# TzuYaoHuang/WaterLily.jl

Measured on AMD Instinct MI355X. Metric: cells*steps/sec (3D TGV) ; smoother HBM GB/s vs peak, higher is better.
Workload: dtype f32; 1 GPU; 3D Taylor-Green vortex 512^3 Float32, wall-bounded, Re=1600, NoBody, remeasure=false (BASELINE configs[4] domain on 1 GPU); size=512, resjac=630, resjac_redo=0

## Files before the change

waterlily.jl_amd/csrc/wl_common.hpp:

```cpp
#pragma once
#include <functional>
#include <cstdlib>
#include <hip/hip_runtime.h>
#include <stdint.h>

#include <mutex>
#include <string>
#include <vector>

#include "../../include/wlhip.h"
#include "../../include/wlhip_bench.h"

#define WL_WAVE 64
#define WL_BLOCK 256

void wl_set_error(const std::string& s);
#define WL_HIP(call)                                                                      \
  do {                                                                                    \
    hipError_t e__ = (call);                                                              \
    if (e__ != hipSuccess) {                                                              \
      wl_set_error(std::string(#call) + ": " + hipGetErrorString(e__));                   \
      return (int)e__;                                                                    \
    }                                                                                     \
  } while (0)
// ... 121 lines not shown
  RedWs w; char* b = (char*)base;
  w.pa = (double*)b; w.pb = (double*)(b + (size_t)WL_MAXPART * 8); w.pm = (float*)(b + (size_t)WL_MAXPART * 16);
  w.res_d = (double*)(b + (size_t)WL_MAXPART * 20); w.res_f = (float*)(b + (size_t)WL_MAXPART * 20 + 64);
  return w;
}

struct WlCtx {
  bool inited = false;
  int device = 0;
  void* red = nullptr;
  double* h_d = nullptr;
  float* h_f = nullptr;
};
WlCtx& wl_ctx();
int wl_ctx_ensure();

struct WlProf {
  bool on = false;
  bool only_roofline = false;
  struct Slot { std::vector<hipEvent_t> a, b; size_t used = 0; };
  Slot slot[WL_PROF_NSLOTS];
};
WlProf& wl_prof();
struct ProfScope {
  int id; hipStream_t s; bool active; size_t idx;
  ProfScope(int id_, hipStream_t s_);
  ~ProfScope();
};

struct BcFold { int on; float U[3];
                const float* proj_x = nullptr; int proj_done = 0;
                int usub = 0;
                const float* go = nullptr;
                const float* dt_dev = nullptr; };

namespace wl {
struct ConstL { int on; float c[3]; float Dt[27]; float iDt[27]; };
#ifdef __HIPCC__
__device__ __forceinline__ float wl_cl_coef(int Ia, int Na, float c) { return (Ia <= 2 || Ia >= Na) ? 0.f : c; }
__device__ __forceinline__ int wl_cl_cnt(int Ia, int Na) { return ((Ia <= 2 || Ia >= Na) ? 0 : 1) + ((Ia + 1 <= 2 || Ia + 1 >= Na) ? 0 : 1); }
#endif
int check_const_L(const float* L, const GridX& g, ConstL* out, int* dev_flag, hipStream_t s);
int const_plane_range(const float* L, const GridX& g, const float* c, int* za, int* zb, hipStream_t s);
int fill(float* a, float v, size_t n, hipStream_t s);
int scale(float* a, float s_, size_t n, hipStream_t s);
int div_scalar(float* a, float s_, size_t n, hipStream_t s);
int div_scalar_to(float* out, const float* in, float s_, size_t n, hipStream_t s);
int sum_dev(const float* a, size_t n, const RedWs& ws, int slot, hipStream_t s);
int l1_linf_dev(const float* a, size_t n, const RedWs& ws, int slot_d, int slot_f, hipStream_t s);
int max_dev(const float* a, size_t n, const RedWs& ws, int slot_f, hipStream_t s);
int dot_dev(const float* a, const float* b, size_t n, const RedWs& ws, int slot, hipStream_t s);
int read_results(const RedWs& ws, double* hd, int nd, float* hf, int nf, hipStream_t s);
int read_results_overlapped(const RedWs& ws, double* hd, int nd, float* hf, int nf, hipStream_t s, hipEvent_t copied, const std::function<int()>& queue_behind);
std::mutex& wl_read_mutex();

int bc_vec(float* a, const GridX& g, const float* U, int saveexit, unsigned per, hipStream_t s);
int bc_per_scalar(float* a, const GridX& g, unsigned per, hipStream_t s);
int conv_diff(float* r, const float* u, float* Phi, const GridX& g, float nu, unsigned per, int scheme, hipStream_t s);
int conv_diff_bdim(float* f, const float* u_adv, float* Phi, const float* u0, const float* mu0, float* u_out, const GridX& g, float nu, unsigned per, int scheme,
                   float dt, float pre, float post, const ConstL& cl, hipStream_t s, int ka = -(1 << 30), int kb = 1 << 30, bool q1 = true, BcFold* fold = nullptr);
int conv_q1(float* Phi, const float* u, const GridX& g, float nu, unsigned per, int scheme, hipStream_t s);
bool conv_z_ok(const GridX& g, unsigned per);
int conv_diff_z(float* f, const float* u_adv, const float* u0, const float* mu0, float* u_out, const GridX& g, float nu, int scheme, float dt, float pre, float post, hipStream_t s);
int bdim(float* u, const float* u0, float* f, const float* V, const float* mu0, const float* mu1, const GridX& g, float dt, float pre, float post, hipStream_t s);
int accelerate(float* r, const GridX& g, const float* a, hipStream_t s);
int sgs(float* f, float* sigma, const float* u, const GridX& g, float Cs, float Delta, hipStream_t s);
int bc_vec_fn(float* a, const float* Ub, const GridX& g, int saveexit, unsigned per, hipStream_t s);
// ... 97 lines not shown
```

waterlily.jl_amd/csrc/wl_poisson.hip:

```cpp
#include <vector>

#include "wl_common.hpp"
#include "wl_bcfold.hpp"
#include "wl_pdefer.hpp"

namespace {

__device__ __forceinline__ bool cell_ij(const GridX& g, long m, int& i, int& j) {
  if (m >= g.sz) return false;
  j = (int)(m / g.nx);
  i = (int)(m - (long)j * g.nx);
  return true;
}
__device__ __forceinline__ bool interior_ij(const GridX& g, int i, int j) { return i >= 1 && i <= g.nx - 2 && j >= 1 && j <= g.ny - 2; }

template <int D>
__device__ __forceinline__ float Ax(const GridX& g, long o, const float* __restrict__ L, const float* __restrict__ Dg, const float* __restrict__ x) {
  float s = x[o] * Dg[o];
  s += (x[o - 1] * L[o] + x[o + 1] * L[o + 1]);
  s += (x[o - g.sy] * L[g.cs + o] + x[o + g.sy] * L[g.cs + o + g.sy]);
  if (D == 3) s += (x[o - g.sz] * L[2 * g.cs + o] + x[o + g.sz] * L[2 * g.cs + o + g.sz]);
  return s;
}

// ... 255 lines not shown
      if (bc.usub) {
        if (i0 == 0 || i0 == g.nx - 2) a0.y = bc.U[0];
        if (j == 1) a1 = make_float2(bc.U[1], bc.U[1]);
        if (j + 1 == g.ny - 1) a1p = make_float2(bc.U[1], bc.U[1]);
        if (g.gk + k == 1) a2 = make_float2(bc.U[2], bc.U[2]);
        if (g.gk + k + 1 == g.gnz - 1) a2p = make_float2(bc.U[2], bc.U[2]);
      }
      const float uxn0 = a0.x - lx0 * (xc.x - xl), uxp0 = a0.y - lx1 * (xc.y - xc.x);
      const float uyn0 = a1.x - ly * (xc.x - xym.x), uyp0 = a1p.x - lyp * (xyp.x - xc.x);
      const float uzn0 = a2.x - lz * (xc.x - xzm.x), uzp0 = a2p.x - lzp * (xzp.x - xc.x);
      const float uxn1 = a0.y - lx1 * (xc.y - xc.x), uxp1 = axr - lx2 * (xr - xc.y);
      const float uyn1 = a1.y - ly * (xc.y - xym.y), uyp1 = a1p.y - lyp * (xyp.y - xc.y);
      const float uzn1 = a2.y - lz * (xc.y - xzm.y), uzp1 = a2p.y - lzp * (xzp.y - xc.y);
      if (in0) { sg0 = 0.f; sg0 += (fmaxf(0.f, uxp0) + fmaxf(0.f, -uxn0)); sg0 += (fmaxf(0.f, uyp0) + fmaxf(0.f, -uyn0)); sg0 += (fmaxf(0.f, uzp0) + fmaxf(0.f, -uzn0)); }
      if (in1) { sg1 = 0.f; sg1 += (fmaxf(0.f, uxp1) + fmaxf(0.f, -uxn1)); sg1 += (fmaxf(0.f, uyp1) + fmaxf(0.f, -uyn1)); sg1 += (fmaxf(0.f, uzp1) + fmaxf(0.f, -uzn1)); }
      const float va[3] = {uxn0, uyn0, uzn0}, vb[3] = {uxn1, uyn1, uzn1};
      const bool plain0 = !bc.on || wl_bc_fold_plain(g, i0, j, k), plain1 = !bc.on || wl_bc_fold_plain(g, i0 + 1, j, k);
      if (in0 && in1 && plain0 && plain1) { pl_st2(uout, o, make_float2(va[0], vb[0])); pl_st2(uout, g.cs + o, make_float2(va[1], vb[1])); pl_st2(uout, 2 * g.cs + o, make_float2(va[2], vb[2])); }
      else {
        if (in0) { if (plain0) { uout[o] = va[0]; uout[g.cs + o] = va[1]; uout[2 * g.cs + o] = va[2]; } else wl_bc_fold_store(uout, g, i0, j, k, va, bc.U); }
        if (in1) { if (plain1) { uout[o + 1] = vb[0]; uout[g.cs + o + 1] = vb[1]; uout[2 * g.cs + o + 1] = vb[2]; } else wl_bc_fold_store(uout, g, i0 + 1, j, k, vb, bc.U); }
      }
      if (store_sigma) { if (in0) sigma[o] = sg0; if (in1) sigma[o + 1] = sg1; }
    }
    if (want) {
      if (!in0) sg0 = sigma[o];
      if (!in1) sg1 = sigma[o + 1];
      mx = fmaxf(sg0, sg1);
    }
  }
  mx = block_max(mx);
  if (threadIdx.x == 0) atomicMax(reinterpret_cast<int*>(pmax) + (blockIdx.x & (WL_ENC_SLOTS - 1)), wl_enc_f(mx));
}

__global__ void k_fin_max_enc(const int* __restrict__ p, float* __restrict__ om) {
  float mx = -INFINITY;
  for (int q = threadIdx.x; q < WL_ENC_SLOTS; q += WL_BLOCK) { const int k = p[q]; if (k != (int)0x80000000) mx = fmaxf(mx, wl_dec_f(k)); }
  mx = block_max(mx); if (threadIdx.x == 0) *om = mx;
}
__global__ void k_fin_max2(const float* __restrict__ pmax, int n, float* __restrict__ om) {
  float mx = -INFINITY, m1 = -INFINITY, m2 = -INFINITY, m3 = -INFINITY;
  int q = threadIdx.x;
  for (; q + 3 * WL_BLOCK < n; q += 4 * WL_BLOCK) { mx = fmaxf(mx, pmax[q]); m1 = fmaxf(m1, pmax[q + WL_BLOCK]); m2 = fmaxf(m2, pmax[q + 2 * WL_BLOCK]); m3 = fmaxf(m3, pmax[q + 3 * WL_BLOCK]); }
  for (; q < n; q += WL_BLOCK) mx = fmaxf(mx, pmax[q]);
  mx = fmaxf(fmaxf(mx, m1), fmaxf(m2, m3));
  mx = block_max(mx); if (threadIdx.x == 0) *om = mx;
}
template <int D>
__global__ void k_check_const_L(GridX g, const float* __restrict__ L, float c0, float c1, float c2, int* __restrict__ flag) {
  int i, j; long m; int pz;
  wl_tile(g, m, pz);
  if (!cell_ij(g, m, i, j)) return;
  const int k = pz;
  const int Kj = (D == 3) ? g.gk + k + 1 : 1;
  if (D == 3 && (Kj < 1 || Kj > g.gnz)) return;
  if (D == 3 && g.nz != g.gnz && (k < g.k0 - 1 || k > g.k1)) return;
  const long o = m + (long)k * g.sz;
  const float c[3] = {c0, c1, c2};
  const int I[3] = {i + 1, j + 1, Kj};
  const int N[3] = {g.nx, g.ny, (D == 3) ? g.gnz : 1};
  bool bad = false;
  for (int a = 0; a < D; a++) {
    const float want = (I[a] <= 2 || I[a] >= N[a]) ? 0.f : c[a];
    bad = bad || (L[(long)a * g.cs + o] != want);
  }
  if (bad) atomicOr(flag, 1);
// ... 648 lines not shown
  hipLaunchKernelGGL(k_final_sum, dim3(1), dim3(WL_BLOCK), 0, s, ws.pa, (int)grid.x, ws.res_d + 0);
  WL_LAUNCH_CHECK(); return 0;
}
#define DSEL2(D, CLF, KERN, ...)                                                                                     \
  do { if ((D) == 3) { if (CLF) hipLaunchKernelGGL((KERN<3, 1>), __VA_ARGS__); else hipLaunchKernelGGL((KERN<3, 0>), __VA_ARGS__); } \
       else { if (CLF) hipLaunchKernelGGL((KERN<2, 1>), __VA_ARGS__); else hipLaunchKernelGGL((KERN<2, 0>), __VA_ARGS__); } } while (0)
int div_residual(float* z, float* xout, float* r, const float* x, const float* u, const float* L, const float* Dg, const float* iD, const GridX& g, float dt, const RedWs& ws, const ConstL& cl, hipStream_t s) {
  const int zc = wl_march_chunk(g, g.nz);
  dim3 grid = wl_plane_grid(g, wl_march_slots(g.nz, zc));
  DSEL2(g.D, cl.on, k_div_residual, grid, dim3(WL_BLOCK), 0, s, g, z, xout, r, x, u, L, Dg, iD, dt, ws.pa, cl, zc, 0, g.nz);
  hipLaunchKernelGGL(k_final_sum, dim3(1), dim3(WL_BLOCK), 0, s, ws.pa, (int)grid.x, ws.res_d + 0);
  WL_LAUNCH_CHECK(); return 0;
}
int div_residual_split(float* z, float* xout, float* r, const float* x, const float* u, const float* L, const float* Dg, const float* iD, const GridX& g, float dt, const RedWs& ws,
                       const ConstL& near, const ConstL& far, int na, int nb, hipStream_t s) {
  const int lo[3] = {0, na, nb}, hi[3] = {na, nb, g.nz};
  int off = 0;
  for (int q = 0; q < 3; q++) {
    const int np = hi[q] - lo[q];
    if (np <= 0) continue;
    const ConstL& cl = q == 1 ? near : far;
    const int zc = wl_march_chunk(g, np);
    dim3 grid = wl_plane_grid(g, wl_march_slots(np, zc));
    if (off + (int)grid.x > WL_MAXPART) { wl_set_error("div_residual_split: too many partial sums"); return WL_EINVAL; }
    DSEL2(g.D, cl.on, k_div_residual, grid, dim3(WL_BLOCK), 0, s, g, z, xout, r, x, u, L, Dg, iD, dt, ws.pa + off, cl, zc, lo[q], hi[q]);
    off += (int)grid.x;
  }
  hipLaunchKernelGGL(k_final_sum, dim3(1), dim3(WL_BLOCK), 0, s, ws.pa, off, ws.res_d + 0);
  WL_LAUNCH_CHECK(); return 0;
}
static int tail_pair_bits() { static const int v = wl_exp_int("WL_TAIL_PAIR", 2); return v; }
static int tail_pair() { return tail_pair_bits() & 1; }
static int tail_lin(int bit) { static const int v = wl_exp_int("WL_TAIL_LIN", 1); return (v >> bit) & 1; }
int project_unscale(float* u, const float* L, const float* x, float* pout, const GridX& g, float dt, const ConstL& cl, hipStream_t s, const BcFold* fold) {
  return project_unscale(u, L, x, pout, g, dt, cl, s, fold, false);
}
int project_unscale(float* u, const float* L, const float* x, float* pout, const GridX& g, float dt, const ConstL& cl, hipStream_t s, const BcFold* fold, bool skip_p) {
  const int lin = tail_lin(0) && g.D == 3;
  const int zc = lin ? 1 : wl_march_chunk(g, g.nz);
  BcFold bc{0, {0.f, 0.f, 0.f}};
  if (fold && fold->on && g.D == 3 && g.nz == g.gnz && g.nx >= 6 && g.ny >= 6 && g.nz >= 6) bc = *fold;
  bc.go = fold ? fold->go : nullptr;
  if (tail_pair() && lin && cl.on && (g.nx & 1) == 0 && g.k0 >= 1) {
    if (skip_p) hipLaunchKernelGGL(k_project_unscale2<0>, dim3(pl_grid(g, g.nz)), dim3(WL_BLOCK), 0, s, g, u, x, pout, dt, cl, 0, g.nz, bc);
    else hipLaunchKernelGGL(k_project_unscale2<1>, dim3(pl_grid(g, g.nz)), dim3(WL_BLOCK), 0, s, g, u, x, pout, dt, cl, 0, g.nz, bc);
    WL_LAUNCH_CHECK(); return 0;
  }
  if (skip_p) {
    if (!(g.D == 3 && cl.on)) { wl_set_error("project_unscale: the tail without the p store needs a 3-D constant-coefficient level"); return WL_EINVAL; }
    hipLaunchKernelGGL((k_project_unscale<3, 1, 0>), wl_plane_grid(g, wl_march_slots(g.nz, zc)), dim3(WL_BLOCK), 0, s, g, u, L, x, pout, dt, cl, zc, 0, g.nz, bc, lin);
    WL_LAUNCH_CHECK(); return 0;
  }
  DSEL2(g.D, cl.on, k_project_unscale, wl_plane_grid(g, wl_march_slots(g.nz, zc)), dim3(WL_BLOCK), 0, s, g, u, L, x, pout, dt, cl, zc, 0, g.nz, bc, lin);
  WL_LAUNCH_CHECK(); return 0;
}
int project_unscale_split(float* u, const float* L, const float* x, float* pout, const GridX& g, float dt, const ConstL& near, const ConstL& far, int na, int nb, hipStream_t s) {
  const int lo[3] = {0, na, nb}, hi[3] = {na, nb, g.nz};
  for (int q = 0; q < 3; q++) {
    const int np = hi[q] - lo[q];
    if (np <= 0) continue;
    const ConstL& cl = q == 1 ? near : far;
    const int zc = wl_march_chunk(g, np);
    DSEL2(g.D, cl.on, k_project_unscale, wl_plane_grid(g, wl_march_slots(np, zc)), dim3(WL_BLOCK), 0, s, g, u, L, x, pout, dt, cl, zc, lo[q], hi[q], BcFold{0, {0.f, 0.f, 0.f}}, 0);
  }
  WL_LAUNCH_CHECK(); return 0;
}
__global__ void k_decide(const double* __restrict__ res_d, float* __restrict__ res_f, double r1tol, double rinftol, double ninside, int check_head, int slot_d, int slot_f, int out_slot) {
  const float rnew = (float)res_d[slot_d], rinf = res_f[slot_f];
  const bool ok = (double)rnew < r1tol && (double)rinf < rinftol;
  const bool head_due = check_head == 2 || (check_head == 1 && wl_shift_due(res_d[0], ninside));
  res_f[out_slot] = head_due ? -1.f : (ok ? 1.f : 0.f);
}
int decide_converged(const RedWs& ws, double r1tol, double rinftol, double ninside, int check_head, int slot_d, int slot_f, int out_slot, hipStream_t s) {
  hipLaunchKernelGGL(k_decide, dim3(1), dim3(1), 0, s, (const double*)ws.res_d, ws.res_f, r1tol, rinftol, ninside, check_head, slot_d, slot_f, out_slot);
  WL_LAUNCH_CHECK(); return 0;
}
bool project_cfl_pair_path(const GridX& g, const ConstL& cl) { return (tail_pair_bits() & 2) && g.D == 3 && cl.on && (g.nx & 1) == 0 && g.k0 >= 1 && g.k1 <= g.nz - 1; }
int project_cfl(float* uout, const float* uin, const float* L, const float* x, float* pout, float* sigma, const GridX& g, float dt, const ConstL& cl, const RedWs& ws, int slot_f, hipStream_t s, int store_sigma, const BcFold* fold) {
  return project_cfl(uout, uin, L, x, pout, sigma, g, dt, cl, ws, slot_f, s, store_sigma, fold, false);
}
int project_cfl(float* uout, const float* uin, const float* L, const float* x, float* pout, float* sigma, const GridX& g, float dt, const ConstL& cl, const RedWs& ws, int slot_f, hipStream_t s, int store_sigma, const BcFold* fold,
                bool skip_p) {
  if (uout == uin) { wl_set_error("project_cfl: output aliases input"); return WL_EINVAL; }
  int kfirst = 0, klast = 1;
  if (g.D == 3) { kfirst = (g.gk + g.k0 == 1) ? g.k0 - 1 : g.k0; klast = (g.gk + g.k1 == g.gnz - 1) ? g.k1 + 1 : g.k1; }
  BcFold bc{0, {0.f, 0.f, 0.f}};
  if (fold && fold->on && g.D == 3 && g.nz == g.gnz && g.nx >= 6 && g.ny >= 6 && g.nz >= 6) bc = *fold;
  bc.go = fold ? fold->go : nullptr;
  if (bc.go && !project_cfl_pair_path(g, cl)) { wl_set_error("project_cfl: a tail queued ahead of the convergence read needs the two-cells-per-thread form"); return WL_EINVAL; }
  if (fold && fold->usub && !(bc.on && project_cfl_pair_path(g, cl))) { wl_set_error("project_cfl: deferred BC! needs the folded two-cells-per-thread tail"); return WL_EINVAL; }
  if (skip_p && !project_cfl_pair_path(g, cl)) { wl_set_error("project_cfl: the tail without the p store needs the two-cells-per-thread form"); return WL_EINVAL; }
  if (project_cfl_pair_path(g, cl)) {
    hipLaunchKernelGGL(k_enc_init, dim3(1), dim3(WL_ENC_SLOTS), 0, s, reinterpret_cast<int*>(ws.pm));
    if (skip_p) hipLaunchKernelGGL(k_project_cfl2<0>, dim3(pl_grid(g, g.nz)), dim3(WL_BLOCK), 0, s, g, uout, uin, x, pout, sigma, dt, cl, kfirst, klast, ws.pm, 0, g.nz, store_sigma, bc);
    else hipLaunchKernelGGL(k_project_cfl2<1>, dim3(pl_grid(g, g.nz)), dim3(WL_BLOCK), 0, s, g, uout, uin, x, pout, sigma, dt, cl, kfirst, klast, ws.pm, 0, g.nz, store_sigma, bc);
    hipLaunchKernelGGL(k_fin_max_enc, dim3(1), dim3(WL_BLOCK), 0, s, reinterpret_cast<const int*>(ws.pm), ws.res_f + slot_f);
    WL_LAUNCH_CHECK(); return 0;
  }
  const int lin = tail_lin(1) && g.D == 3;
  const int zc = lin ? 1 : wl_march_chunk(g, g.nz);
  const dim3 grid = wl_plane_grid(g, wl_march_slots(g.nz, zc));
  if (lin) hipLaunchKernelGGL(k_enc_init, dim3(1), dim3(WL_ENC_SLOTS), 0, s, reinterpret_cast<int*>(ws.pm));
  DSEL2(g.D, cl.on, k_project_cfl, grid, dim3(WL_BLOCK), 0, s, g, uout, uin, L, x, pout, sigma, dt, cl, zc, kfirst, klast, ws.pm, 0, g.nz, store_sigma, bc, lin);
  if (lin) hipLaunchKernelGGL(k_fin_max_enc, dim3(1), dim3(WL_BLOCK), 0, s, reinterpret_cast<const int*>(ws.pm), ws.res_f + slot_f);
  else hipLaunchKernelGGL(k_fin_max2, dim3(1), dim3(WL_BLOCK), 0, s, ws.pm, (int)grid.x, ws.res_f + slot_f);
  WL_LAUNCH_CHECK(); return 0;
}
int project_cfl_split(float* uout, const float* uin, const float* L, const float* x, float* pout, float* sigma, const GridX& g, float dt, const ConstL& near, const ConstL& far,
                      int na, int nb, const RedWs& ws, int slot_f, hipStream_t s, int store_sigma) {
  if (uout == uin) { wl_set_error("project_cfl: output aliases input"); return WL_EINVAL; }
  int kfirst = 0, klast = 1;
  if (g.D == 3) { kfirst = (g.gk + g.k0 == 1) ? g.k0 - 1 : g.k0; klast = (g.gk + g.k1 == g.gnz - 1) ? g.k1 + 1 : g.k1; }
  const int lo[3] = {0, na, nb}, hi[3] = {na, nb, g.nz};
  int off = 0;
  for (int q = 0; q < 3; q++) {
    const int np = hi[q] - lo[q];
    if (np <= 0) continue;
    const ConstL& cl = q == 1 ? near : far;
    const int zc = wl_march_chunk(g, np);
    const dim3 grid = wl_plane_grid(g, wl_march_slots(np, zc));
    if (off + (int)grid.x > WL_MAXPART) { wl_set_error("project_cfl_split: too many partial maxima"); return WL_EINVAL; }
    DSEL2(g.D, cl.on, k_project_cfl, grid, dim3(WL_BLOCK), 0, s, g, uout, uin, L, x, pout, sigma, dt, cl, zc, kfirst, klast, ws.pm + off, lo[q], hi[q], store_sigma, BcFold{0, {0.f, 0.f, 0.f}}, 0);
    off += (int)grid.x;
  }
  hipLaunchKernelGGL(k_fin_max2, dim3(1), dim3(WL_BLOCK), 0, s, ws.pm, off, ws.res_f + slot_f);
  WL_LAUNCH_CHECK(); return 0;
}
// ... 172 lines not shown
```

waterlily.jl_amd/csrc/wl_sim.hip:

```cpp
#include <cmath>
#include <cstring>
#include <utility>
#include <vector>

#include "wl_common.hpp"
#include <algorithm>
#include "wl_mg.hpp"
#include "wl_body.hpp"
#include "wl_pdefer.hpp"

namespace {
__device__ __forceinline__ bool cell_ij(const GridX& g, long m, int& i, int& j) {
  if (m >= g.sz) return false;
  j = (int)(m / g.nx);
  i = (int)(m - (long)j * g.nx);
  return true;
}
__device__ __forceinline__ bool interior_ij(const GridX& g, int i, int j) { return i >= 1 && i <= g.nx - 2 && j >= 1 && j <= g.ny - 2; }

template <int D>
__global__ void k_apply_tgv(GridX g, float* __restrict__ u, float kx, float ky, float kz) {
  int i, j; long m; int pz;
  wl_tile(g, m, pz);
  if (!cell_ij(g, m, i, j)) return;
// ... 370 lines not shown
          WL_TRY(sync_u(s));
          WL_TRY(wl::conv_diff_z(store_f ? f : nullptr, u, u0, mu0, us, G, d.nu, d.scheme, dt.back(), 1.f, 0.5f, s));
          WL_TRY(wl::conv_q1(sigma, u, G, d.nu, d.perdir_mask, d.scheme, s));
        } else { WL_TRY(conv_fused(u, us, 1.f, 0.5f, s)); fused_conv = true; } }
      std::swap(u, us);
      if (d.exitBC) WL_TRY(copy_exit_face(u, us, s));
      return fused_conv ? bc_u_or_defer(true, s) : bc_u(s);
    }
    { ProfScope pc(WL_PROF_CONVDIFF, s); WL_TRY(conv_only(u, s)); }
    WL_TRY(sgs_udf(u, s));
    if (forcing) WL_TRY(wl::accelerate(f, G, acc1, s));
    WL_TRY(bdim_step(1.f, 0.5f, s));
    return bc_u(s);
  }
  int itmx = 32;
  bool use_resjac = true;
  bool use_headspec = true;
  bool resjac_force_redo = false;
  bool redo_unannounced = false;
  long n_tailfuse = 0;
  long n_resjac = 0, n_resjac_redo = 0;
  int resjac_redo_run = 0;
  bool resjac_backoff = false;
  int p_shell = -1;
  bool use_fuse_cfl = true;
  bool cfl_done = false;
  static constexpr int CFL_SLOT = 5;
  bool use_tailspec = true;
  long n_tailspec = 0, n_tailspec_armed = 0;
  bool use_pdefer = true;
  float p_scale_pending = 0.f;
  long n_pdefer = 0;
  float* p_home = nullptr;
  bool pdefer_ok() const { return use_pdefer && in_step && !sgs_model && !forcing && !d.has_body && head_fused_ok(); }
  int materialise_p(hipStream_t s) {
    if (p_scale_pending == 0.f) return 0;
    const float dp = p_scale_pending; p_scale_pending = 0.f;
    WL_TRY(wl::div_scalar_to(ps, p, dp, (size_t)G.cs, s));
    std::swap(p, ps); mg->lv[0].x = p;
    return 0;
  }
  int project(float w, hipStream_t s, bool with_cfl = false, bool defer_tail = false, bool more_follow = false) {
    const float dtl = w * dt.back();
    cfl_done = false;
    if (p_scale_pending != 0.f && !head_fused_ok()) WL_TRY(materialise_p(s));
    WL_TRY(sync_u(s));
    if (bc_deferred && !head_fused_ok()) WL_TRY(flush_bc(s));
    if (ps && use_fuse_p && !(comm && d.perdir_mask)) {
      WL_TRY(wl::bc_per_scalar(p, G, d.perdir_mask, s));
      wl_mg::Level& l0 = mg->lv[0];
      bool head_done = false;
      double pre_r1 = 0.0; float pre_rinf = 0.f;
      bool solved = false;
      const bool split = l0.part && mg->use_zsplit && !comm;
      const int zm = 4, zna = split ? std::max(l0.g.k0, l0.za - zm) : 0, znb = split ? std::min(l0.g.k1, l0.zb + zm + 1) : 0;
      int tail_kind = 0;
      bool tail_stood = false;
      bool tail_skips_p = false;
      auto skip_p_now = [&]() -> bool {
        if (!pdefer_ok()) return false;
        if (with_cfl) return more_follow;
        if (!defer_tail) return false;
        return !p_home || more_follow || p == p_home;
      };
      auto launch_tail = [&](const float* go) -> int {
        tail_skips_p = false;
        if (with_cfl && use_fuse_cfl && us && !d.exitBC && !d.perdir_mask) {
          tail_kind = 1;
          if (split) { WL_TRY(flush_bc(s)); WL_TRY(wl::project_cfl_split(us, u, mu0, p, ps, sigma, G, dtl, l0.cl, l0.clp, zna, znb, mg->ws, CFL_SLOT, s, store_f ? 1 : 0)); }
          else {
            BcFold fr = fold_req(1);
            if (bc_deferred && !(fr.on && wl::project_cfl_pair_path(G, l0.cl))) WL_TRY(flush_bc(s));
            fr.usub = bc_deferred ? 1 : 0;
            fr.go = go;
            tail_skips_p = wl::project_cfl_pair_path(G, l0.cl) && skip_p_now();
            WL_TRY(wl::project_cfl(us, u, mu0, p, ps, sigma, G, dtl, l0.cl, mg->ws, CFL_SLOT, s, store_f ? 1 : 0, &fr, tail_skips_p)); bc_folded = fr.on != 0;
          }
        } else if (split) { tail_kind = 2; WL_TRY(wl::project_unscale_split(u, mu0, p, ps, G, dtl, l0.cl, l0.clp, zna, znb, s)); }
        else if (defer_tail && tailfuse_ok()) {
          tail_kind = 3;
          tail_skips_p = skip_p_now();
          if (!tail_skips_p) WL_TRY(wl::div_scalar_to(ps, p, dtl, (size_t)G.cs, s));
        }
        else { tail_kind = 2; BcFold fr = fold_req(1); fr.go = go; tail_skips_p = skip_p_now(); WL_TRY(wl::project_unscale(u, mu0, p, ps, G, dtl, l0.cl, s, &fr, tail_skips_p)); bc_folded = fr.on != 0; }
        return 0;
      };
      const bool tail_gateable = !split && !(defer_tail && tailfuse_ok()) &&
                                 (!(with_cfl && use_fuse_cfl && us && !d.exitBC && !d.perdir_mask) || (wl::project_cfl_pair_path(G, l0.cl) && (!bc_deferred || fold_req(1).on)));
      if (use_resjac && !resjac_backoff && !d.exitBC && !store_f && !d.perdir_mask && !l0.part && mg->defer_shift && mg->lv.size() > 1 && wl::resjac_ok(G, l0.cl) &&
          (!comm || (l0.dist && mg->x_halo_depth >= 2))) {
        { ProfScope pr(WL_PROF_RESIDUAL, s);
          if (comm) p_shell = 1;
          if (p_shell < 0) p_shell = (wl::shell_nonzero(p, G, (int*)(mg->ws.res_f + 7), s) || wl::shell_nonzero(ps, G, (int*)(mg->ws.res_f + 7), s)) ? 1 : 0;
          WL_TRY(wl::resjac(ps, l0.eps, p, u, G, dtl, 1.f, l0.cl, mg->ws, 1, 0, s, p_shell != 0, bc_deferred ? d.uBC : nullptr, p_scale_pending)); }
        if (use_headspec && !comm && itmx >= 1) {
          std::swap(p, ps); l0.x = p;
          std::swap(l0.r, l0.eps);
          mg->jacobi0_done = true;
          struct SpecClear { wl_mg* m; ~SpecClear() { m->spec_tail = nullptr; m->spec_check_head = 0; } } spec_clear{mg};
          if (use_tailspec && tail_gateable) { mg->spec_tail = launch_tail; mg->spec_check_head = resjac_force_redo ? 2 : 1; n_tailspec_armed++; }
          WL_TRY(mg->solve(2e-3, itmx, nullptr, nullptr, nullptr, s, true, nullptr, nullptr));
          tail_stood = mg->tail_stood; if (tail_stood) n_tailspec++;
          const bool due = mg->head_decided ? mg->head_due : (resjac_force_redo || wl_shift_due(mg->first_hd0, (double)wl_ninside_global(mg->lv[0].g)));
          if (!due) { head_done = true; solved = true; n_resjac++; resjac_redo_run = 0; }
          else {
            std::swap(l0.r, l0.eps); std::swap(p, ps); l0.x = p;
            mg->n.pop_back(); mg->jacobi0_done = false;
            n_resjac_redo++;
            if (!resjac_force_redo && ++resjac_redo_run >= 3) resjac_backoff = true;
          }
        } else {
        WL_TRY(wl::combine_results(comm, mg->ws, s));
        double hd2[2]; WL_TRY(wl::read_results(mg->ws, hd2, 2, &pre_rinf, 1, s));
        const double sr = hd2[0]; pre_r1 = hd2[1];
        if (!wl_shift_due(sr, (double)wl_ninside_global(mg->lv[0].g)) && !resjac_force_redo) {
          std::swap(p, ps); l0.x = p;
          std::swap(l0.r, l0.eps);
          mg->jacobi0_done = true; head_done = true; n_resjac++; resjac_redo_run = 0;
        } else {
          n_resjac_redo++;
          if (!resjac_force_redo && ++resjac_redo_run >= 3) resjac_backoff = true;
        }
        }
      }
      if (head_done) p_scale_pending = 0.f;
      if (!head_done) {
        WL_TRY(materialise_p(s));
        WL_TRY(flush_bc(s));
        ProfScope pr(WL_PROF_RESIDUAL, s);
        if (l0.part && mg->use_zsplit && !comm) {
          const int m = 4, na = std::max(l0.g.k0, l0.za - m), nb = std::min(l0.g.k1, l0.zb + m + 1);
          WL_TRY(wl::div_residual_split(store_f ? sigma : nullptr, ps, l0.r, p, u, mu0, l0.D, l0.iD, G, dtl, mg->ws, l0.cl, l0.clp, na, nb, s));
        } else WL_TRY(wl::div_residual(store_f ? sigma : nullptr, ps, l0.r, p, u, mu0, l0.D, l0.iD, G, dtl, mg->ws, l0.cl, s));
      }
      if (!head_done) { std::swap(p, ps); l0.x = p; }
      if (!solved) WL_TRY(mg->solve(2e-3, itmx, nullptr, nullptr, nullptr, s, true, head_done ? &pre_r1 : nullptr, head_done ? &pre_rinf : nullptr));
      if (!tail_stood) WL_TRY(launch_tail(nullptr));
      if (tail_kind == 3) {
        bc_deferred = false;
        proj_pending = p;
        if (tail_skips_p) { p_scale_pending = dtl; n_pdefer++; }
        else { std::swap(p, ps); l0.x = p; }
        n_tailfuse++;
        return 0;
      }
      if (tail_kind == 1) {
        bc_deferred = false;
        WL_TRY(wl::combine_results(comm, mg->ws, s));
        std::swap(u, us); cfl_done = true;
      }
      if (tail_skips_p) { p_scale_pending = dtl; n_pdefer++; }
      else { std::swap(p, ps); l0.x = p; }
      bc_deferred = false;
      return bc_u(s);
    }
    WL_TRY(materialise_p(s));
    WL_TRY(flush_bc(s));
    WL_TRY(wl::div_scale(sigma, p, u, G, dtl, s));
    WL_TRY(mg->solve(2e-3, itmx, nullptr, nullptr, nullptr, s));
    WL_TRY(wl::project(u, mu0, p, G, s));
    WL_TRY(wl::div_scalar(p, dtl, (size_t)G.cs, s));
    return bc_u(s);
  }
  bool use_lazydt = true, dt_pending = false;
  hipEvent_t ev_dt = nullptr;
  bool lazydt_ok() const {
    return use_lazydt && in_step && !comm && us && !d.has_body && !forcing && !sgs_model && !use_convz && !d.exitBC && !d.perdir_mask && !store_f && wl::conv_flux_on() &&
           wl::conv_tile_ok(G, d.perdir_mask, G.k1 - G.k0) && mg->lv[0].cl.on;
  }
  int cfl(hipStream_t s, bool more_follow = false) {
    if (!cfl_done) { WL_TRY(sync_u(s)); WL_TRY(wl::cfl_dev(u, sigma, G, mg->ws, CFL_SLOT, s)); WL_TRY(wl::combine_results(comm, mg->ws, s)); }
    cfl_done = false;
    if (more_follow && lazydt_ok()) {
      hipLaunchKernelGGL(k_dt_from_cfl, dim3(1), dim3(1), 0, s, mg->ws.res_f, CFL_SLOT, CFL_SLOT + 1, d.nu);
      dt_pending = true;
      return 0;
    }
    float hf6[CFL_SLOT + 1]; WL_TRY(wl::read_results(mg->ws, nullptr, 0, hf6, CFL_SLOT + 1, s)); const float mx = hf6[CFL_SLOT];
    dt.push_back(std::fmin(10.f, 1.0f / (mx + 5 * d.nu)));
    return 0;
  }
  int mom_step(hipStream_t s, bool more_follow = false) {
    const int rc = mom_step_body(s, more_follow);
// ... 220 lines not shown
  const std::string n(name);
  if (n == "convz") { s->use_convz = value != 0; return 0; }
  if (n == "fused_smoother") { s->mg->use_fused = value != 0; return 0; }
  if (n == "store_eps") { s->mg->store_eps = value != 0; return 0; }
  if (n == "constl") { s->mg->use_constl = value != 0; return s->mg->update(0); }
  if (n == "tail") { s->mg->use_tail = value != 0; return 0; }
  if (n == "tail_lds") { wl::tail_lds_enable(value); return 0; }
  if (n == "xdefer") { s->mg->use_xdefer = value != 0; return 0; }
  if (n == "overlap_smooth") { s->mg->overlap_smooth = value != 0; return 0; }
  if (n == "body_tile") { wl::conv_body_tile_enable(value); return 0; }
  if (n == "skip_fill") { s->mg->skip_fill = value != 0; return 0; }
  if (n == "defer_shift") { s->mg->defer_shift = value != 0; return 0; }
  if (n == "zsplit") {
    s->mg->use_zsplit = value != 0; s->mg->zsplit_min = value == 2 ? 0 : (value >= 4 ? (long)value << 20 : 16L << 20); return 0;
  }
  if (n == "hybrid") { s->use_hybrid = value != 0; return 0; }
  if (n == "farmask") { s->use_farmask = value != 0; return 0; }
  if (n == "store_f") { s->store_f = value != 0; return 0; }
  if (n == "overlap") { WL_TRY(s->sync_u(0)); s->use_overlap = value != 0; return 0; }
  if (n == "fuse_cfl") { s->use_fuse_cfl = value != 0; return 0; }
  if (n == "jacobi_march") { wl::jacobi_march_enable(value); return 0; }
  if (n == "convm") { wl::conv_march_enable(value); return 0; }
  if (n == "deep_halo") { s->mg->deep_halo = value != 0; return 0; }
  if (n == "x_halo") { if (value < 1 || value > s->G.k0) { wl_set_error("x_halo: 1 .. ghost depth of the slab"); return WL_EINVAL; } s->mg->x_halo_depth = value; return 0; }
  if (n == "bcfold") { s->use_bcfold = value; return 0; }
  if (n == "resjac") { s->use_resjac = value != 0; s->resjac_force_redo = value == 2 || value == 3; s->redo_unannounced = value == 3; return 0; }
  if (n == "resjac_min") { wl::resjac_enable(1, value); return 0; }
  if (n == "convt_min") { wl::conv_tile_min(value); return 0; }
  if (n == "lazydt") { s->use_lazydt = value != 0; return 0; }
  if (n == "tailspec") { s->use_tailspec = value != 0; return 0; }
  if (n == "headspec") { s->use_headspec = value != 0; return 0; }
  if (n == "bcdefer") { s->use_bcdefer = value != 0; return 0; }
  if (n == "pdefer") { s->use_pdefer = value != 0; return 0; }
  if (n == "tailfuse") { s->use_tailfuse = value != 0; return 0; }
  if (n == "convf") { wl::conv_flux_enable(value != 0); return 0; }
  if (n == "convt") { wl::conv_tile_enable(value != 0, value > 1 ? value : 0); return 0; }
  if (n == "pair") { wl::gsrb_pair_enable(value); return 0; }
  if (n == "fuse_p") { s->use_fuse_p = value != 0; return 0; }
  if (n == "zsplit_par") { s->mg->par_ranges = value != 0; return 0; }
  if (n == "itmx") { if (value < 1) { wl_set_error("itmx must be >= 1"); return WL_EINVAL; } s->itmx = value; return 0; }
  wl_set_error("unknown option " + n); return WL_EINVAL;
}
int wl_sim_update(wl_sim* s, void* st) { s->resjac_backoff = false; s->resjac_redo_run = 0; WL_TRY(s->refresh_body_mask(wl_stream(st))); return s->mg->update(wl_stream(st)); }

long wl_launch_count(void) { return g_wl_launches; }
int wl_reset_process_options(void) {
  wl::resjac_enable(1, 6L << 20); wl::conv_tile_min(2048); wl::conv_tile_enable(1, 0); wl::conv_flux_enable(1); wl::tail_lds_enable(1); wl::conv_body_tile_enable(1);
  wl::gsrb_pair_enable(1); wl::jacobi_march_enable(1); wl::conv_march_enable(0);
  return 0;
}
int wl_sim_counter(wl_sim* s, const char* name, long* out) {
  WL_CHECK(s && name && out, "bad argument");
  const std::string n(name);
  if (n == "resjac") { *out = s->n_resjac; return 0; }
  if (n == "resjac_redo") { *out = s->n_resjac_redo; return 0; }
  if (n == "resjac_backoff") { *out = s->resjac_backoff ? 1 : 0; return 0; }
  if (n == "tailfuse") { *out = s->n_tailfuse; return 0; }
  if (n == "bcdefer") { *out = s->n_bcdefer; return 0; }
  if (n == "pdefer") { *out = s->n_pdefer; return 0; }
  if (n == "tailspec") { *out = s->n_tailspec; return 0; }
  if (n == "tailspec_armed") { *out = s->n_tailspec_armed; return 0; }
  if (n == "xdefer") { *out = s->mg->last_xdefer; return 0; }
  wl_set_error("unknown counter " + n); return WL_EINVAL;
}
int wl_sim_set_forcing(wl_sim* s, const float* U1, const float* a0, const float* a1) {
  const int D = s->d.D;
  if (U1) for (int c = 0; c < D; c++) s->d.uBC[c] = U1[c];
  s->forcing = a0 != nullptr || a1 != nullptr;
  for (int c = 0; c < 3; c++) { s->acc0[c] = (a0 && c < D) ? a0[c] : 0.f; s->acc1[c] = (a1 && c < D) ? a1[c] : 0.f; }
  return 0;
}
int wl_sim_set_sgs(wl_sim* s, int model, float Cs, float Delta) {
  WL_CHECK(s, "null wl_sim"); WL_CHECK(model == 0 || model == 1, "wl_sim_set_sgs: model must be 0 (off) or 1 (Smagorinsky-Lilly)");
  if (model) {
    if (s->d.D != 3) { wl_set_error("wl_sim_set_sgs: the Smagorinsky model is built for 3-D flows only"); return WL_EINVAL; }
    if (s->comm) { wl_set_error("wl_sim_set_sgs: z-slab handles are not supported (single domain only)"); return WL_EINVAL; }
  }
  s->sgs_model = model; s->sgs_Cs = Cs; s->sgs_Delta = Delta;
  return 0;
}
int wl_accelerate(float* r, const wl_grid* g, const float* a, void* st) {
  WL_CHECK(wl_grid_ok(g) && a, "bad argument"); WL_TRY(wl_ctx_ensure());
  return wl::accelerate(r, gx(*g), a, wl_stream(st));
}
int wl_sim_mom_step(wl_sim* s, void* st) { return s->mom_step(wl_stream(st)); }
int wl_sim_mom_steps(wl_sim* s, int n, void* st) {
  WL_CHECK(s && n >= 0, "bad argument");
  for (int k = 0; k < n; k++) WL_TRY(s->mom_step(wl_stream(st), k + 1 < n));
  return 0;
}
int wl_sim_dt(const wl_sim* s, float* out, int cap) { const int n = (int)s->dt.size(); for (int k = 0; k < n && k < cap; k++) out[k] = s->dt[(size_t)k]; return n; }
float wl_sim_dt_last(const wl_sim* s) { return s->dt.back(); }
// ... 157 lines not shown
```

Before: 14.51 billion cells*steps/s.

## Add four-cells-per-thread projection tail kernel with LDS-staged pressure plane

Adds a new projection/CFL tail kernel in which each thread handles four consecutive cells using float4 loads and stores. The pressure chunk plus its y-halo is staged in shared memory so the x and y neighbours are read from LDS instead of global memory. It is enabled by default through a new tailwide option and is guarded by alignment and shape checks. The aim is fewer memory transactions and better bandwidth use in the once-per-step tail. In exchange it uses LDS and more registers, has more complex boundary handling, and can fall back to the older paired kernel.

```diff
diff --git a/waterlily.jl_amd/csrc/wl_common.hpp b/waterlily.jl_amd/csrc/wl_common.hpp
--- a/waterlily.jl_amd/csrc/wl_common.hpp
+++ b/waterlily.jl_amd/csrc/wl_common.hpp
@@ -177,7 +177,8 @@
                 const float* proj_x = nullptr; int proj_done = 0;
                 int usub = 0;
                 const float* go = nullptr;
-                const float* dt_dev = nullptr; };
+                const float* dt_dev = nullptr;
+                int wide = 0; int* wide_ran = nullptr; };
 
 namespace wl {
 struct ConstL { int on; float c[3]; float Dt[27]; float iDt[27]; };
diff --git a/waterlily.jl_amd/csrc/wl_poisson.hip b/waterlily.jl_amd/csrc/wl_poisson.hip
--- a/waterlily.jl_amd/csrc/wl_poisson.hip
+++ b/waterlily.jl_amd/csrc/wl_poisson.hip
@@ -311,6 +311,130 @@
   mx = block_max(mx);
   if (threadIdx.x == 0) atomicMax(reinterpret_cast<int*>(pmax) + (blockIdx.x & (WL_ENC_SLOTS - 1)), wl_enc_f(mx));
 }
+#define WL_TW_CHUNK (4 * WL_BLOCK)
+__device__ __forceinline__ float4 tw_ld4(const float* __restrict__ p, long o) { return *reinterpret_cast<const float4*>(p + o); }
+__device__ __forceinline__ void tw_st4(float* __restrict__ p, long o, float4 v) { *reinterpret_cast<float4*>(p + o) = v; }
+static inline unsigned tw_nb8(const GridX& g) { const long nb = (g.sz + WL_TW_CHUNK - 1) / WL_TW_CHUNK; return (unsigned)(((nb + 7) >> 3) << 3); }
+static inline unsigned tw_grid(const GridX& g, int nplanes) { return tw_nb8(g) * (unsigned)nplanes; }
+static inline size_t tw_lds_bytes(const GridX& g) { return (size_t)(WL_TW_CHUNK + 2 * g.sy + 8) * sizeof(float); }
+template <int CFL, int SP>
+__global__ void __launch_bounds__(WL_BLOCK) k_project_wide(GridX g, float* __restrict__ uout, const float* __restrict__ uin, const float* __restrict__ x, float* __restrict__ pout,
+                                                              float* __restrict__ sigma, float dt, wl::ConstL cl, int kfirst, int klast, float* __restrict__ pmax, int p0, int p1,
+                                                              int store_sigma, BcFold bc, unsigned nb8) {
+  if (bc.go && !(*bc.go > 0.f)) return;
+  extern __shared__ float4 tw_sh[];
+  float* __restrict__ xs = reinterpret_cast<float*>(tw_sh);
+  const float* __restrict__ ui = CFL ? uin : uout;
+  const unsigned h = blockIdx.x, p = h / nb8;
+  const int k = p0 + (int)p;
+  const long m0 = (long)(h - p * nb8) * WL_TW_CHUNK;
+  float mx = -INFINITY;
+  if (m0 < g.sz && k < p1) {
+    const long ko = (long)k * g.sz;
+    const int sy = (int)g.sy;
+    const long base = (m0 - sy) & ~3L;
+    const bool zin = k >= g.k0 && k < g.k1;
+    if (zin) {
+      const long whi = (m0 + WL_TW_CHUNK + (CFL ? sy : 0) + 3) & ~3L;
+      for (long q = base + 4 * (long)threadIdx.x; q < whi; q += 4 * WL_BLOCK)
+        *reinterpret_cast<float4*>(xs + (q - base)) = (q >= 0 && q < g.sz) ? tw_ld4(x, ko + q) : make_float4(0.f, 0.f, 0.f, 0.f);
+      __syncthreads();
+    }
+    const float lz = wl::wl_cl_coef(g.gk + k + 1, g.gnz, cl.c[2]), lzp = wl::wl_cl_coef(g.gk + k + 2, g.gnz, cl.c[2]);
+    const bool want = CFL && k >= kfirst && k < klast;
+    const long m = m0 + 4 * (long)threadIdx.x;
+    if (m < g.sz) {
+      const long o = ko + m;
+      const int r = (int)(m - base);
+      const float4 xq = zin ? *reinterpret_cast<const float4*>(xs + r) : tw_ld4(x, o);
+      const float X[6] = {zin ? xs[r - 1] : 0.f, xq.x, xq.y, xq.z, xq.w, (CFL && zin) ? xs[r + 4] : 0.f};
+      if (SP) tw_st4(pout, o, make_float4(wl_unscale(xq.x, dt), wl_unscale(xq.y, dt), wl_unscale(xq.z, dt), wl_unscale(xq.w, dt)));
+      const int j0 = (int)(m / g.nx), i0 = (int)(m - (long)j0 * g.nx);
+      int ii[4], jj[4]; bool in[4];
+#pragma unroll
+      for (int c = 0; c < 4; c++) {
+        int i = i0 + c, j = j0;
+        if (i >= g.nx) { i -= g.nx; j++; }
+        ii[c] = i; jj[c] = j;
+        in[c] = zin && i >= 1 && i <= g.nx - 2 && j >= 1 && j <= g.ny - 2;
+      }
+      float sg[4] = {0.f, 0.f, 0.f, 0.f};
+      if (in[0] || in[1] || in[2] || in[3]) {
+        const float2 ym0 = *reinterpret_cast<const float2*>(xs + r - sy), ym1 = *reinterpret_cast<const float2*>(xs + r - sy + 2);
+        const float XYM[4] = {ym0.x, ym0.y, ym1.x, ym1.y};
+        const float4 zmq = tw_ld4(x, o - g.sz);
+        const float XZM[4] = {zmq.x, zmq.y, zmq.z, zmq.w};
+        const float4 a0q = tw_ld4(ui, o), a1q = tw_ld4(ui, g.cs + o), a2q = tw_ld4(ui, 2 * g.cs + o);
+        float A0[5] = {a0q.x, a0q.y, a0q.z, a0q.w, 0.f};
+        const float A1[4] = {a1q.x, a1q.y, a1q.z, a1q.w}, A2[4] = {a2q.x, a2q.y, a2q.z, a2q.w};
+        float XYP[4] = {0.f, 0.f, 0.f, 0.f}, XZP[4] = {0.f, 0.f, 0.f, 0.f}, A1P[4] = {0.f, 0.f, 0.f, 0.f}, A2P[4] = {0.f, 0.f, 0.f, 0.f};
+        if (CFL) {
+          const float2 yp0 = *reinterpret_cast<const float2*>(xs + r + sy), yp1 = *reinterpret_cast<const float2*>(xs + r + sy + 2);
+          XYP[0] = yp0.x; XYP[1] = yp0.y; XYP[2] = yp1.x; XYP[3] = yp1.y;
+          const float4 zpq = tw_ld4(x, o + g.sz), a2pq = tw_ld4(ui, 2 * g.cs + o + g.sz);
+          XZP[0] = zpq.x; XZP[1] = zpq.y; XZP[2] = zpq.z; XZP[3] = zpq.w;
+          A2P[0] = a2pq.x; A2P[1] = a2pq.y; A2P[2] = a2pq.z; A2P[3] = a2pq.w;
+          A0[4] = ui[o + 4];
+          const float2 b0 = *reinterpret_cast<const float2*>(ui + g.cs + o + sy), b1 = *reinterpret_cast<const float2*>(ui + g.cs + o + sy + 2);
+          A1P[0] = b0.x; A1P[1] = b0.y; A1P[2] = b1.x; A1P[3] = b1.y;
+        }
+        float V[4][3]; bool plain[4];
+#pragma unroll
+        for (int c = 0; c < 4; c++) {
+          const int i = ii[c], j = jj[c];
+          const float xc = X[c + 1];
+          const float lx = wl::wl_cl_coef(i + 1, g.nx, cl.c[0]), ly = wl::wl_cl_coef(j + 1, g.ny, cl.c[1]);
+          float a0 = A0[c], a0n = A0[c + 1], a1 = A1[c], a1p = A1P[c], a2 = A2[c], a2p = A2P[c];
+          if (CFL && bc.usub) {
+            if (i == 1) a0 = bc.U[0];
+            if (i + 2 == g.nx) a0n = bc.U[0];
+            if (j == 1) a1 = bc.U[1];
+            if (j + 2 == g.ny) a1p = bc.U[1];
+            if (g.gk + k == 1) a2 = bc.U[2];
+            if (g.gk + k + 2 == g.gnz) a2p = bc.U[2];
+          }
+          const float uxn = a0 - lx * (xc - X[c]);
+          const float uyn = a1 - ly * (xc - XYM[c]);
+          const float uzn = a2 - lz * (xc - XZM[c]);
+          V[c][0] = uxn; V[c][1] = uyn; V[c][2] = uzn;
+          if (CFL) {
+            const float lxp = wl::wl_cl_coef(i + 2, g.nx, cl.c[0]), lyp = wl::wl_cl_coef(j + 2, g.ny, cl.c[1]);
+            const float uxp = a0n - lxp * (X[c + 2] - xc);
+            const float uyp = a1p - lyp * (XYP[c] - xc);
+            const float uzp = a2p - lzp * (XZP[c] - xc);
+            if (in[c]) { float s = 0.f; s += (fmaxf(0.f, uxp) + fmaxf(0.f, -uxn)); s += (fmaxf(0.f, uyp) + fmaxf(0.f, -uyn)); s += (fmaxf(0.f, uzp) + fmaxf(0.f, -uzn)); sg[c] = s; }
+          }
+          plain[c] = in[c] && (!bc.on || wl_bc_fold_plain(g, i, j, k));
+        }
+        if (plain[0] && plain[1] && plain[2] && plain[3]) {
+          tw_st4(uout, o, make_float4(V[0][0], V[1][0], V[2][0], V[3][0]));
+          tw_st4(uout, g.cs + o, make_float4(V[0][1], V[1][1], V[2][1], V[3][1]));
+          tw_st4(uout, 2 * g.cs + o, make_float4(V[0][2], V[1][2], V[2][2], V[3][2]));
+        } else {
+#pragma unroll
+          for (int c = 0; c < 4; c++) {
+            if (!in[c]) continue;
+            if (plain[c]) { uout[o + c] = V[c][0]; uout[g.cs + o + c] = V[c][1]; uout[2 * g.cs + o + c] = V[c][2]; }
+            else wl_bc_fold_store(uout, g, ii[c], jj[c], k, V[c], bc.U);
+          }
+        }
+        if (CFL && store_sigma) {
+#pragma unroll
+          for (int c = 0; c < 4; c++) if (in[c]) sigma[o + c] = sg[c];
+        }
+      }
+      if (want) {
+#pragma unroll
+        for (int c = 0; c < 4; c++) if (!in[c]) sg[c] = sigma[o + c];
+        mx = fmaxf(mx, fmaxf(fmaxf(sg[0], sg[1]), fmaxf(sg[2], sg[3])));
+      }
+    }
+  }
+  if (CFL) {
+    mx = block_max(mx);
+    if (threadIdx.x == 0) atomicMax(reinterpret_cast<int*>(pmax) + (blockIdx.x & (WL_ENC_SLOTS - 1)), wl_enc_f(mx));
+  }
+}
 
 __global__ void k_fin_max_enc(const int* __restrict__ p, float* __restrict__ om) {
   float mx = -INFINITY;
@@ -1025,6 +1149,7 @@
 static int tail_pair_bits() { static const int v = wl_exp_int("WL_TAIL_PAIR", 2); return v; }
 static int tail_pair() { return tail_pair_bits() & 1; }
 static int tail_lin(int bit) { static const int v = wl_exp_int("WL_TAIL_LIN", 1); return (v >> bit) & 1; }
+static bool project_wide_path(const GridX& g, const ConstL& cl, const void* a, const void* b, const void* c, const void* d = nullptr, const void* e = nullptr);
 int project_unscale(float* u, const float* L, const float* x, float* pout, const GridX& g, float dt, const ConstL& cl, hipStream_t s, const BcFold* fold) {
   return project_unscale(u, L, x, pout, g, dt, cl, s, fold, false);
 }
@@ -1034,6 +1159,13 @@
   BcFold bc{0, {0.f, 0.f, 0.f}};
   if (fold && fold->on && g.D == 3 && g.nz == g.gnz && g.nx >= 6 && g.ny >= 6 && g.nz >= 6) bc = *fold;
   bc.go = fold ? fold->go : nullptr;
+  if (fold && fold->wide && lin && project_wide_path(g, cl, u, x, skip_p ? nullptr : pout)) {
+    if (fold->wide_ran) *fold->wide_ran = 1;
+    const dim3 grid(tw_grid(g, g.nz));
+    if (skip_p) hipLaunchKernelGGL((k_project_wide<0, 0>), grid, dim3(WL_BLOCK), tw_lds_bytes(g), s, g, u, nullptr, x, pout, nullptr, dt, cl, 0, 0, nullptr, 0, g.nz, 0, bc, tw_nb8(g));
+    else hipLaunchKernelGGL((k_project_wide<0, 1>), grid, dim3(WL_BLOCK), tw_lds_bytes(g), s, g, u, nullptr, x, pout, nullptr, dt, cl, 0, 0, nullptr, 0, g.nz, 0, bc, tw_nb8(g));
+    WL_LAUNCH_CHECK(); return 0;
+  }
   if (tail_pair() && lin && cl.on && (g.nx & 1) == 0 && g.k0 >= 1) {
     if (skip_p) hipLaunchKernelGGL(k_project_unscale2<0>, dim3(pl_grid(g, g.nz)), dim3(WL_BLOCK), 0, s, g, u, x, pout, dt, cl, 0, g.nz, bc);
     else hipLaunchKernelGGL(k_project_unscale2<1>, dim3(pl_grid(g, g.nz)), dim3(WL_BLOCK), 0, s, g, u, x, pout, dt, cl, 0, g.nz, bc);
@@ -1067,6 +1199,13 @@
 int decide_converged(const RedWs& ws, double r1tol, double rinftol, double ninside, int check_head, int slot_d, int slot_f, int out_slot, hipStream_t s) {
   hipLaunchKernelGGL(k_decide, dim3(1), dim3(1), 0, s, (const double*)ws.res_d, ws.res_f, r1tol, rinftol, ninside, check_head, slot_d, slot_f, out_slot);
   WL_LAUNCH_CHECK(); return 0;
+}
+static bool project_wide_path(const GridX& g, const ConstL& cl, const void* a, const void* b, const void* c, const void* d, const void* e) {
+  if (!(g.D == 3 && cl.on && (g.nx & 1) == 0 && g.nx >= 8 && g.ny >= 4 && (g.sz & 3) == 0 && g.k0 >= 1 && g.k1 <= g.nz - 1)) return false;
+  if (tw_lds_bytes(g) > 48 * 1024 || (long)tw_nb8(g) * g.nz > 0x7fffffffL) return false;
+  const void* ptr[5] = {a, b, c, d, e};
+  for (int q = 0; q < 5; q++) if ((reinterpret_cast<uintptr_t>(ptr[q]) & 15) != 0) return false;
+  return true;
 }
 bool project_cfl_pair_path(const GridX& g, const ConstL& cl) { return (tail_pair_bits() & 2) && g.D == 3 && cl.on && (g.nx & 1) == 0 && g.k0 >= 1 && g.k1 <= g.nz - 1; }
 int project_cfl(float* uout, const float* uin, const float* L, const float* x, float* pout, float* sigma, const GridX& g, float dt, const ConstL& cl, const RedWs& ws, int slot_f, hipStream_t s, int store_sigma, const BcFold* fold) {
@@ -1085,7 +1224,13 @@
   if (skip_p && !project_cfl_pair_path(g, cl)) { wl_set_error("project_cfl: the tail without the p store needs the two-cells-per-thread form"); return WL_EINVAL; }
   if (project_cfl_pair_path(g, cl)) {
     hipLaunchKernelGGL(k_enc_init, dim3(1), dim3(WL_ENC_SLOTS), 0, s, reinterpret_cast<int*>(ws.pm));
-    if (skip_p) hipLaunchKernelGGL(k_project_cfl2<0>, dim3(pl_grid(g, g.nz)), dim3(WL_BLOCK), 0, s, g, uout, uin, x, pout, sigma, dt, cl, kfirst, klast, ws.pm, 0, g.nz, store_sigma, bc);
+    if (fold && fold->wide && project_wide_path(g, cl, uout, uin, x, sigma, skip_p ? nullptr : pout)) {
+      if (fold->wide_ran) *fold->wide_ran = 1;
+      const dim3 grid(tw_grid(g, g.nz));
+      if (skip_p) hipLaunchKernelGGL((k_project_wide<1, 0>), grid, dim3(WL_BLOCK), tw_lds_bytes(g), s, g, uout, uin, x, pout, sigma, dt, cl, kfirst, klast, ws.pm, 0, g.nz, store_sigma, bc, tw_nb8(g));
+      else hipLaunchKernelGGL((k_project_wide<1, 1>), grid, dim3(WL_BLOCK), tw_lds_bytes(g), s, g, uout, uin, x, pout, sigma, dt, cl, kfirst, klast, ws.pm, 0, g.nz, store_sigma, bc, tw_nb8(g));
+    }
+    else if (skip_p) hipLaunchKernelGGL(k_project_cfl2<0>, dim3(pl_grid(g, g.nz)), dim3(WL_BLOCK), 0, s, g, uout, uin, x, pout, sigma, dt, cl, kfirst, klast, ws.pm, 0, g.nz, store_sigma, bc);
     else hipLaunchKernelGGL(k_project_cfl2<1>, dim3(pl_grid(g, g.nz)), dim3(WL_BLOCK), 0, s, g, uout, uin, x, pout, sigma, dt, cl, kfirst, klast, ws.pm, 0, g.nz, store_sigma, bc);
     hipLaunchKernelGGL(k_fin_max_enc, dim3(1), dim3(WL_BLOCK), 0, s, reinterpret_cast<const int*>(ws.pm), ws.res_f + slot_f);
     WL_LAUNCH_CHECK(); return 0;
diff --git a/waterlily.jl_amd/csrc/wl_sim.hip b/waterlily.jl_amd/csrc/wl_sim.hip
--- a/waterlily.jl_amd/csrc/wl_sim.hip
+++ b/waterlily.jl_amd/csrc/wl_sim.hip
@@ -426,6 +426,8 @@
   float p_scale_pending = 0.f;
   long n_pdefer = 0;
   float* p_home = nullptr;
+  bool use_tailwide = true;
+  long n_tailwide = 0;
   bool pdefer_ok() const { return use_pdefer && in_step && !sgs_model && !forcing && !d.has_body && head_fused_ok(); }
   int materialise_p(hipStream_t s) {
     if (p_scale_pending == 0.f) return 0;
@@ -450,6 +452,7 @@
       const int zm = 4, zna = split ? std::max(l0.g.k0, l0.za - zm) : 0, znb = split ? std::min(l0.g.k1, l0.zb + zm + 1) : 0;
       int tail_kind = 0;
       bool tail_stood = false;
+      bool tail_wide = false;
       bool tail_skips_p = false;
       auto skip_p_now = [&]() -> bool {
         if (!pdefer_ok()) return false;
@@ -458,7 +461,7 @@
         return !p_home || more_follow || p == p_home;
       };
       auto launch_tail = [&](const float* go) -> int {
-        tail_skips_p = false;
+        tail_skips_p = false; tail_wide = false;
         if (with_cfl && use_fuse_cfl && us && !d.exitBC && !d.perdir_mask) {
           tail_kind = 1;
           if (split) { WL_TRY(flush_bc(s)); WL_TRY(wl::project_cfl_split(us, u, mu0, p, ps, sigma, G, dtl, l0.cl, l0.clp, zna, znb, mg->ws, CFL_SLOT, s, store_f ? 1 : 0)); }
@@ -468,7 +471,8 @@
             fr.usub = bc_deferred ? 1 : 0;
             fr.go = go;
             tail_skips_p = wl::project_cfl_pair_path(G, l0.cl) && skip_p_now();
-            WL_TRY(wl::project_cfl(us, u, mu0, p, ps, sigma, G, dtl, l0.cl, mg->ws, CFL_SLOT, s, store_f ? 1 : 0, &fr, tail_skips_p)); bc_folded = fr.on != 0;
+            int ran = 0; fr.wide = use_tailwide ? 1 : 0; fr.wide_ran = &ran;
+            WL_TRY(wl::project_cfl(us, u, mu0, p, ps, sigma, G, dtl, l0.cl, mg->ws, CFL_SLOT, s, store_f ? 1 : 0, &fr, tail_skips_p)); bc_folded = fr.on != 0; tail_wide = ran != 0;
           }
         } else if (split) { tail_kind = 2; WL_TRY(wl::project_unscale_split(u, mu0, p, ps, G, dtl, l0.cl, l0.clp, zna, znb, s)); }
         else if (defer_tail && tailfuse_ok()) {
@@ -476,7 +480,9 @@
           tail_skips_p = skip_p_now();
           if (!tail_skips_p) WL_TRY(wl::div_scalar_to(ps, p, dtl, (size_t)G.cs, s));
         }
-        else { tail_kind = 2; BcFold fr = fold_req(1); fr.go = go; tail_skips_p = skip_p_now(); WL_TRY(wl::project_unscale(u, mu0, p, ps, G, dtl, l0.cl, s, &fr, tail_skips_p)); bc_folded = fr.on != 0; }
+        else { tail_kind = 2; BcFold fr = fold_req(1); fr.go = go; tail_skips_p = skip_p_now();
+               int ran = 0; fr.wide = use_tailwide ? 1 : 0; fr.wide_ran = &ran;
+               WL_TRY(wl::project_unscale(u, mu0, p, ps, G, dtl, l0.cl, s, &fr, tail_skips_p)); bc_folded = fr.on != 0; tail_wide = ran != 0; }
         return 0;
       };
       const bool tail_gateable = !split && !(defer_tail && tailfuse_ok()) &&
@@ -543,6 +549,7 @@
         WL_TRY(wl::combine_results(comm, mg->ws, s));
         std::swap(u, us); cfl_done = true;
       }
+      if (tail_wide) n_tailwide++;
       if (tail_skips_p) { p_scale_pending = dtl; n_pdefer++; }
       else { std::swap(p, ps); l0.x = p; }
       bc_deferred = false;
@@ -829,6 +836,7 @@
   if (n == "headspec") { s->use_headspec = value != 0; return 0; }
   if (n == "bcdefer") { s->use_bcdefer = value != 0; return 0; }
   if (n == "pdefer") { s->use_pdefer = value != 0; return 0; }
+  if (n == "tailwide") { s->use_tailwide = value != 0; return 0; }
   if (n == "tailfuse") { s->use_tailfuse = value != 0; return 0; }
   if (n == "convf") { wl::conv_flux_enable(value != 0); return 0; }
   if (n == "convt") { wl::conv_tile_enable(value != 0, value > 1 ? value : 0); return 0; }
@@ -855,6 +863,7 @@
   if (n == "tailfuse") { *out = s->n_tailfuse; return 0; }
   if (n == "bcdefer") { *out = s->n_bcdefer; return 0; }
   if (n == "pdefer") { *out = s->n_pdefer; return 0; }
+  if (n == "tailwide") { *out = s->n_tailwide; return 0; }
   if (n == "tailspec") { *out = s->n_tailspec; return 0; }
   if (n == "tailspec_armed") { *out = s->n_tailspec_armed; return 0; }
   if (n == "xdefer") { *out = s->mg->last_xdefer; return 0; }
```

Result: faster. 14.73 billion cells*steps/s, median of 6 (+1.6%).
